# idiap/IdiapTTS

Measured on AMD Instinct MI355X. Metric: acoustic frames/sec (train), higher is better.
Workload: dtype f32

## Files before the change

idiaptts_amd/csrc/gemm_ring.h:

```cpp
#pragma once
#include <hip/hip_runtime.h>
#include <stdint.h>

#ifndef RING_DBG
#define RING_DBG 0
#endif

namespace itts {
namespace ring {

typedef float f32x16 __attribute__((ext_vector_type(16)));
typedef float f32x4 __attribute__((ext_vector_type(4)));
typedef __attribute__((address_space(3))) char* lds_char_p;

constexpr int RBK = 32;
constexpr int SLOT_BYTES = 192 * 128;
#ifndef RING_NSLOT
#define RING_NSLOT 3
#endif
constexpr int NSLOT = RING_NSLOT;
constexpr int RED_BYTES = 2 * 256 * 4;
constexpr int LDS_BYTES = NSLOT * SLOT_BYTES + RED_BYTES;
constexpr int PIECES = 6;
constexpr int THREADS = 512;

enum { EPI_STORE = 0, EPI_BIAS_ACT = 1, EPI_DACT = 2, EPI_MSE = 3 };
enum { ACT_NONE = 0, ACT_TANH = 1, ACT_RELU = 2 };

struct Args {
  const float* A;
  const float* B;
  float* C;
  const float* bias;
  const float* aux;
  const uint8_t* row_valid;
  double* loss_partial;
  float* bias_part;
  uint64_t* stamps;
  int64_t slab_stride;
  int64_t bias_part_stride;
  int lda, ldb, ldc, ldaux;
  int M;
  int N;
  int K;
  int kchunk;
  int splitk;
  int tiles_m, tiles_n;
  int gn;
  int act;
  float gscale;
};

__device__ __forceinline__ float fast_tanhf(float z) {
  const float a = fabsf(z);
  const float z2 = z * z;
  const float poly = z * (1.f + z2 * (-0.33333334f + z2 * (0.13333334f + z2 * (-0.053968254f +
                                                                              z2 * 0.021869488f))));
  const float e = __expf(2.f * a);
  const float big = copysignf(1.f - 2.f * __builtin_amdgcn_rcpf(e + 1.f), z);
  return a < 0.25f ? poly : big;
}

__device__ __forceinline__ __amdgpu_buffer_rsrc_t make_rsrc(const void* p, uint32_t bytes) {
  return __builtin_amdgcn_make_buffer_rsrc(const_cast<void*>(p), 0, (int)bytes, 0x00020000);
}

__device__ __forceinline__ void dma_piece(__amdgpu_buffer_rsrc_t rsrc, uint32_t voff, uint32_t soff, uint32_t dst) {
  asm volatile("s_nop 4\n\ts_mov_b32 m0, %3\n\ts_nop 0\n\tbuffer_load_dwordx4 %0, %1, %2 offen lds"
               :
               : "v"(voff), "s"(rsrc), "s"(soff), "s"(dst)
               : "memory");
}

__device__ __forceinline__ void lds_barrier() {
  asm volatile("s_waitcnt lgkmcnt(0)" ::: "memory");
  __builtin_amdgcn_s_barrier();
  asm volatile("" ::: "memory");
}
__device__ __forceinline__ void step_barrier() {
  if (!(RING_DBG & 2)) __builtin_amdgcn_s_barrier();
  asm volatile("" ::: "memory");
}

template <bool ROW, int BT>
__device__ __forceinline__ float4 read_frag(const char* tile, uint32_t a0, int g) {
  if (ROW) {
    return *reinterpret_cast<const float4*>(tile + (a0 ^ (uint32_t)(g << 5)));
  } else {
    const float* p = reinterpret_cast<const float*>(tile + a0) + g * 8 * BT;
    return make_float4(p[0], p[BT], p[2 * BT], p[3 * BT]);
  }
}
template <bool ROW, int BT>
__device__ __forceinline__ uint32_t frag_base(int o, int lane) {
  const int r = lane & 31, h = lane >> 5;
  if (ROW) {
    const int row = o + r;
    return (uint32_t)(row * 128 + ((((row >> 1) & 7) ^ h) << 4));
  } else {
    return (uint32_t)((4 * h * BT + o + r) * 4);
  }
}

struct Tile {
  int m0, n0, z, tn;
  int kbeg, klen, nk;
};

template <bool GROUPED>
__device__ __forceinline__ Tile decode_tile(const Args& g, int t, int bmt, int bnt) {
  Tile c;
  const int per_z = g.tiles_m * g.tiles_n;
  c.z = t / per_z;
  const int rem = t - c.z * per_z;
  int tm;
  if (!GROUPED) {
    tm = rem / g.tiles_n;
    c.tn = rem - tm * g.tiles_n;
  } else {
    const int per_group = g.tiles_m * g.gn;
    const int grp = rem / per_group;
    const int rem2 = rem - grp * per_group;
    const int left = g.tiles_n - grp * g.gn;
    const int width = left < g.gn ? left : g.gn;
    tm = rem2 / width;
    c.tn = grp * g.gn + (rem2 - tm * width);
  }
  c.m0 = tm * bmt;
  c.n0 = c.tn * bnt;
  c.kbeg = c.z * g.kchunk;
  const int kend = c.kbeg + g.kchunk < g.K ? c.kbeg + g.kchunk : g.K;
  c.klen = kend - c.kbeg;
  c.nk = (c.klen + RBK - 1) / RBK;
  return c;
}

struct Walk {
  int first, end, stride;
};
__device__ __forceinline__ Walk my_tiles(const Args& g) {
  const int ntiles = g.tiles_m * g.tiles_n * g.splitk;
  const int xcd = blockIdx.x & 7, rank = blockIdx.x >> 3;
  const int q = ntiles >> 3, r8 = ntiles & 7;
  const int xstart = xcd < r8 ? xcd * (q + 1) : r8 * (q + 1) + (xcd - r8) * q;
  Walk w;
  w.first = xstart + rank;
  w.end = xstart + q + (xcd < r8 ? 1 : 0);
  w.stride = ((int)gridDim.x - xcd + 7) >> 3;
  return w;
}

template <bool ROW, int BT>
struct Stream {
  __amdgpu_buffer_rsrc_t rsrc;
  uint32_t soff, step;

  __device__ __forceinline__ void open(const float* P, int ld, int out0, int out_dim, const Tile& c) {
    if (ROW) {
      int rows = out_dim - out0;
      rows = rows < BT ? rows : BT;
      step = RBK * 4;
      rsrc = make_rsrc(P + (int64_t)out0 * ld + c.kbeg, (uint32_t)(((int64_t)(rows - 1) * ld + ((c.klen + 3) & ~3)) * 4));
    } else {
      step = (uint32_t)(RBK * ld * 4);
      rsrc = make_rsrc(P + (int64_t)c.kbeg * ld + out0,
                       (uint32_t)(((int64_t)(c.klen - 1) * ld + ((out_dim - out0 + 3) & ~3)) * 4));
    }
    soff = 0;
  }
  __device__ __forceinline__ void issue(uint32_t v0, uint32_t v1, int ld, uint32_t dst, int part) const {
    constexpr int NP = BT / 32;
    if (ROW) {
      const uint32_t pstep = (uint32_t)(16 * ld * 4);
      uint32_t so = soff + (uint32_t)(part * (NP / 2)) * pstep;
      const uint32_t d = dst + part * NP * 1024;
#pragma unroll
      for (int j = 0; j < NP; j += 2) {
        dma_piece(rsrc, v0, so, d + j * 1024);
        dma_piece(rsrc, v1, so, d + (j + 1) * 1024);
        so += pstep;
      }
    } else {
      const uint32_t pstep = (uint32_t)((256 / BT) * ld * 4);
      uint32_t so = soff + (uint32_t)(part * NP) * pstep;
      const uint32_t d = dst + part * NP * 1024;
#pragma unroll
      for (int j = 0; j < NP; ++j) {
        dma_piece(rsrc, v0, so, d + j * 1024);
        so += pstep;
      }
    }
  }
};
template <bool ROW, int BT>
__device__ __forceinline__ void lane_offsets(int ld, int lane, uint32_t& v0, uint32_t& v1) {
  if (ROW) {
    const int r = lane >> 3, c = lane & 7;
    v0 = (uint32_t)(r * ld * 4 + ((c ^ ((r >> 1) & 7)) << 4));
    v1 = (uint32_t)((8 + r) * ld * 4 + ((c ^ (((8 + r) >> 1) & 7)) << 4));
  } else {
    constexpr int LPR = BT / 4;
    v0 = (uint32_t)((lane / LPR) * ld * 4 + (lane % LPR) * 16);
    v1 = v0;
  }
}

template <int BT>
__device__ __forceinline__ void zero_tail(char* tile, int krem, int tid) {
#pragma unroll
  for (int i = 0; i < BT / 32; ++i) {
    const int idx = tid + 256 * i;
    const int row = idx >> 3, c = idx & 7;
    const int lim = krem - 4 * c;
    if (lim < 4) {
      float4* p = reinterpret_cast<float4*>(tile + row * 128 + ((c ^ ((row >> 1) & 7)) << 4));
      float4 v = *p;
      v.x = lim > 0 ? v.x : 0.f;
      v.y = lim > 1 ? v.y : 0.f;
      v.z = lim > 2 ? v.z : 0.f;
      v.w = 0.f;
      *p = v;
    }
  }
}

template <bool A_ROW, bool B_ROW, int BMT, int BNT, bool GROUPED = false>
__device__ __forceinline__ void loader_wave(const Args& g, char* lds, uint32_t lds0, int lane, bool mse, int part) {
  constexpr int A_BYTES = BMT * 128;
  const Walk w = my_tiles(g);
  uint32_t va0, va1, vb0, vb1;
  lane_offsets<A_ROW, BMT>(g.lda, lane, va0, va1);
  lane_offsets<B_ROW, BNT>(g.ldb, lane, vb0, vb1);
  Stream<A_ROW, BMT> sa;
  Stream<B_ROW, BNT> sb;

  int pt = w.first, pk = 0, pnk = 0;
  uint32_t pdst = lds0;
  bool pvalid = pt < w.end;
  auto open = [&]() {
    const Tile c = decode_tile<GROUPED>(g, pt, BMT, BNT);
    sa.open(g.A, g.lda, c.m0, g.M, c);
    sb.open(g.B, g.ldb, c.n0, g.N, c);
    pnk = c.nk;
    pk = 0;
  };
  auto produce = [&]() {
    if (!(RING_DBG & 1)) {
      sa.issue(va0, va1, g.lda, pdst, part);
      sb.issue(vb0, vb1, g.ldb, pdst + A_BYTES, part);
    }
    pdst = pdst == lds0 + (NSLOT - 1) * SLOT_BYTES ? lds0 : pdst + SLOT_BYTES;
    sa.soff += sa.step;
    sb.soff += sb.step;
    if (++pk == pnk) {
      pt += w.stride;
      pvalid = pt < w.end;
      if (pvalid) open();
    }
  };
  int ahead = 0;
  if (pvalid) {
    open();
    for (int i = 0; i < NSLOT - 1 && pvalid; ++i) { produce(); ++ahead; }
  }
  int ct = w.first, kt = 0, cslot = 0;
  bool have = ct < w.end;
  Tile c{};
  if (have) c = decode_tile<GROUPED>(g, ct, BMT, BNT);
  while (have) {
    if (ahead >= 5) asm volatile("s_waitcnt vmcnt(%0)" ::"n"(4 * PIECES) : "memory");
    else if (ahead == 4) asm volatile("s_waitcnt vmcnt(%0)" ::"n"(3 * PIECES) : "memory");
    else if (ahead == 3) asm volatile("s_waitcnt vmcnt(%0)" ::"n"(2 * PIECES) : "memory");
    else if (ahead == 2) asm volatile("s_waitcnt vmcnt(%0)" ::"n"(PIECES) : "memory");
    else asm volatile("s_waitcnt vmcnt(0)" ::: "memory");
    step_barrier();
    --ahead;
    if (pvalid) { produce(); ++ahead; }
    if ((A_ROW || B_ROW) && kt == c.nk - 1 && (c.klen & (RBK - 1)) != 0) step_barrier();
    cslot = cslot == NSLOT - 1 ? 0 : cslot + 1;
    if (++kt == c.nk) {
      kt = 0;
      ct += w.stride;
      have = ct < w.end;
      if (have) c = decode_tile<GROUPED>(g, ct, BMT, BNT);
    }
  }
  if (w.first < w.end) step_barrier();
  if (mse) step_barrier();
}

template <int ACT>
__device__ __forceinline__ float act1(float z) {
  if (ACT == ACT_TANH) return fast_tanhf(z);
  if (ACT == ACT_RELU) return z > 0.f ? z : 0.f;
  return z;
}
template <int ACT>
__device__ __forceinline__ float dact1(float y) {
  if (ACT == ACT_TANH) return 1.f - y * y;
  if (ACT == ACT_RELU) return y > 0.f ? 1.f : 0.f;
  return 1.f;
}

template <int CTRL>
__device__ __forceinline__ float quad_swap(float v) {
  return __builtin_bit_cast(float, __builtin_amdgcn_update_dpp(0, __builtin_bit_cast(int, v), CTRL, 0xf, 0xf, true));
}
__device__ __forceinline__ float4 quad_transpose(float a0, float a1, float a2, float a3, int lane) {
  const bool odd = lane & 1, hi = lane & 2;
  const float s0 = quad_swap<0xB1>(a0), s1 = quad_swap<0xB1>(a1), s2 = quad_swap<0xB1>(a2), s3 = quad_swap<0xB1>(a3);
  const float x0 = odd ? s1 : a0, x1 = odd ? a1 : s0;
  const float x2 = odd ? s3 : a2, x3 = odd ? a3 : s2;
  const float t0 = quad_swap<0x4E>(x0), t1 = quad_swap<0x4E>(x1), t2 = quad_swap<0x4E>(x2), t3 = quad_swap<0x4E>(x3);
  return make_float4(hi ? t2 : x0, hi ? t3 : x1, hi ? x2 : t0, hi ? x3 : t1);
}

template <int EPI>
__device__ __forceinline__ float4 load_bias(const Args& g, int n0, int wn, int lane) {
  float4 bv = make_float4(0.f, 0.f, 0.f, 0.f);
  if ((EPI == EPI_BIAS_ACT || EPI == EPI_MSE) && g.bias) {
    const int col = n0 + wn * 32 + 4 * ((lane & 31) >> 2);
    const __amdgpu_buffer_rsrc_t rb = make_rsrc(g.bias, (uint32_t)(g.N * 4));
    bv.x = __builtin_bit_cast(float, __builtin_amdgcn_raw_buffer_load_b32(rb, col * 4, 0, 0));
    bv.y = __builtin_bit_cast(float, __builtin_amdgcn_raw_buffer_load_b32(rb, col * 4 + 4, 0, 0));
    bv.z = __builtin_bit_cast(float, __builtin_amdgcn_raw_buffer_load_b32(rb, col * 4 + 8, 0, 0));
    bv.w = __builtin_bit_cast(float, __builtin_amdgcn_raw_buffer_load_b32(rb, col * 4 + 12, 0, 0));
  }
  return bv;
}

template <int EPI, int ACT>
__device__ __forceinline__ void epilogue(const Args& g, const Tile& pc, const f32x16& acc0, const f32x16& acc1,
                                         int wm, int wn, int lane, const float4& bv, double& lsum) {
  const int quad = (lane & 31) >> 2, j = lane & 3, h = lane >> 5;
  const int col = pc.n0 + wn * 32 + 4 * quad;
  const int rloc = wm * 64 + 4 * h + j;
  int rows_valid = g.M - pc.m0;
  rows_valid = rows_valid < 0 ? 0 : rows_valid;
  float* Cb = g.C + (int64_t)pc.z * g.slab_stride + (int64_t)pc.m0 * g.ldc;
  const __amdgpu_buffer_rsrc_t rc = make_rsrc(Cb, (uint32_t)((int64_t)rows_valid * g.ldc * 4));
  const uint32_t cofs = col < g.ldc ? (uint32_t)((rloc * g.ldc + col) * 4) : 0xfffffff0u;
  __amdgpu_buffer_rsrc_t rx = rc;
  uint32_t xofs = 0;
  if (EPI == EPI_DACT || EPI == EPI_MSE) {
    rx = make_rsrc(g.aux + (int64_t)pc.m0 * g.ldaux, (uint32_t)((int64_t)rows_valid * g.ldaux * 4));
    xofs = col < g.ldaux ? (uint32_t)((rloc * g.ldaux + col) * 4) : 0xfffffff0u;
  }
  const bool k0 = col < g.N, k1 = col + 1 < g.N, k2 = col + 2 < g.N, k3 = col + 3 < g.N;
#pragma unroll
  for (int i = 0; i < 2; ++i) {
    const f32x16& a = i == 0 ? acc0 : acc1;
#pragma unroll
    for (int rg = 0; rg < 4; ++rg) {
      const int rl = i * 32 + 8 * rg;
      float4 v = quad_transpose(a[4 * rg], a[4 * rg + 1], a[4 * rg + 2], a[4 * rg + 3], lane);
      if (EPI == EPI_BIAS_ACT) {
        v.x = act1<ACT>(v.x + bv.x); v.y = act1<ACT>(v.y + bv.y);
        v.z = act1<ACT>(v.z + bv.z); v.w = act1<ACT>(v.w + bv.w);
      }
      if (EPI == EPI_DACT) {
        const f32x4 y = __builtin_amdgcn_raw_buffer_load_b128(rx, xofs, rl * g.ldaux * 4, 0);
        v.x *= dact1<ACT>(y[0]); v.y *= dact1<ACT>(y[1]);
        v.z *= dact1<ACT>(y[2]); v.w *= dact1<ACT>(y[3]);
      }
      if (EPI == EPI_MSE) {
        f32x4 t;
        {
          const uint32_t so = (uint32_t)(rl * g.ldaux * 4);
          const uint32_t tofs = (uint32_t)((rloc * g.ldaux + col) * 4);
          t[0] = __builtin_bit_cast(float, __builtin_amdgcn_raw_buffer_load_b32(rx, tofs, so, 0));
          t[1] = __builtin_bit_cast(float, __builtin_amdgcn_raw_buffer_load_b32(rx, tofs + 4, so, 0));
          t[2] = __builtin_bit_cast(float, __builtin_amdgcn_raw_buffer_load_b32(rx, tofs + 8, so, 0));
          t[3] = __builtin_bit_cast(float, __builtin_amdgcn_raw_buffer_load_b32(rx, tofs + 12, so, 0));
        }
        const int row = pc.m0 + rloc + rl;
        const bool ok = row < g.M && g.row_valid[row < g.M ? row : 0] != 0;
        const float d0 = ok && k0 ? (v.x + bv.x) - t[0] : 0.f;
        const float d1 = ok && k1 ? (v.y + bv.y) - t[1] : 0.f;
        const float d2 = ok && k2 ? (v.z + bv.z) - t[2] : 0.f;
        const float d3 = ok && k3 ? (v.w + bv.w) - t[3] : 0.f;
        lsum += (double)d0 * (double)d0;
        lsum += (double)d1 * (double)d1;
        lsum += (double)d2 * (double)d2;
        lsum += (double)d3 * (double)d3;
        v = make_float4(g.gscale * d0, g.gscale * d1, g.gscale * d2, g.gscale * d3);
      }
      f32x4 o;
      o[0] = k0 ? v.x : 0.f;
      o[1] = k1 ? v.y : 0.f;
      o[2] = k2 ? v.z : 0.f;
      o[3] = k3 ? v.w : 0.f;
      const uint32_t vo = col < g.ldc ? cofs + (uint32_t)(rl * g.ldc * 4) : 0xfffffff0u;
      if (RING_DBG & 64) asm volatile("" ::"v"(o[0]), "v"(o[1]), "v"(o[2]), "v"(o[3]));
      else __builtin_amdgcn_raw_buffer_store_b128(o, rc, vo, 0, 0);
    }
  }
}

template <bool A_ROW, bool B_ROW, int EPI, int BMT, int BNT, bool GROUPED = false>
__device__ __forceinline__ void compute_waves(const Args& g, char* lds, int wid, int lane) {
  constexpr int WN = BNT / 32;
  constexpr int A_BYTES = BMT * 128;
  const int wm = wid / WN, wn = wid % WN;
  const int tid = wid * 64 + lane;
  const Walk w = my_tiles(g);
  const uint32_t fa0 = frag_base<A_ROW, BMT>(wm * 64, lane);
  const uint32_t fa1 = frag_base<A_ROW, BMT>(wm * 64 + 32, lane);
  const uint32_t fb0 = frag_base<B_ROW, BNT>(wn * 32, lane);
  float* red = reinterpret_cast<float*>(lds + NSLOT * SLOT_BYTES);
  constexpr bool DO_BIAS = !A_ROW && EPI == EPI_STORE;
  constexpr int BPARTS = 256 / BMT;

  double lsum = 0.0;
  int cslot = 0, redbuf = 0;
  bool pending = false;
  Tile pc{};
  f32x16 acc0, acc1;
#pragma unroll
  for (int r = 0; r < 16; ++r) { acc0[r] = 0.f; acc1[r] = 0.f; }
  float bsum = 0.f;

  int ct = w.first;
  bool have = ct < w.end;
  Tile c{};
  if (have) c = decode_tile<GROUPED>(g, ct, BMT, BNT);
  int kt = 0;
  while (have || pending) {
    step_barrier();
    if (pending) {
      if (DO_BIAS && g.bias_part != nullptr && pc.tn == 0) {
        const float* rb = red + (redbuf ^ 1) * 256;
        if (tid < BMT && pc.m0 + tid < g.M) {
          float s = rb[tid];
#pragma unroll
          for (int p = 1; p < BPARTS; ++p) s += rb[tid + p * BMT];
          g.bias_part[(int64_t)pc.z * g.bias_part_stride + pc.m0 + tid] = s;
        }
      }
      if (RING_DBG & 8) {
        float t = 0.f;
        for (int r = 0; r < 16; ++r) t += acc0[r] + acc1[r];
        if (t == 1.2345f) g.C[0] = t;
      } else {
        const float4 bv = load_bias<EPI>(g, pc.n0, wn, lane);
        if (EPI == EPI_STORE || g.act == ACT_NONE) epilogue<EPI, ACT_NONE>(g, pc, acc0, acc1, wm, wn, lane, bv, lsum);
        else if (g.act == ACT_TANH) epilogue<EPI, ACT_TANH>(g, pc, acc0, acc1, wm, wn, lane, bv, lsum);
        else epilogue<EPI, ACT_RELU>(g, pc, acc0, acc1, wm, wn, lane, bv, lsum);
      }
      pending = false;
    }
    if (!have) break;

    char* tA = lds + cslot * SLOT_BYTES;
    char* tB = tA + A_BYTES;
    if ((A_ROW || B_ROW) && kt == c.nk - 1 && (c.klen & (RBK - 1)) != 0) {
      if (A_ROW) zero_tail<BMT>(tA, c.klen & (RBK - 1), tid);
      if (B_ROW) zero_tail<BNT>(tB, c.klen & (RBK - 1), tid);
      lds_barrier();
    }
    if (DO_BIAS && g.bias_part != nullptr && c.tn == 0) {
      constexpr int KP = RBK / BPARTS;
      const float* ctile = reinterpret_cast<const float*>(tA) + (tid / BMT) * KP * BMT + tid % BMT;
#pragma unroll
      for (int kk = 0; kk < KP; ++kk) bsum += ctile[kk * BMT];
    }
#pragma unroll
    for (int kg = 0; kg < 4; ++kg) {
      float4 a0, a1, b0;
      if (RING_DBG & 16) {
        a0 = make_float4(1.f + kg, 2.f, 3.f, 4.f); a1 = a0; b0 = a0;
        asm volatile("" : "+v"(a0.x), "+v"(a1.x), "+v"(b0.x));
      } else {
        a0 = read_frag<A_ROW, BMT>(tA, fa0, kg);
        a1 = read_frag<A_ROW, BMT>(tA, fa1, kg);
        b0 = read_frag<B_ROW, BNT>(tB, fb0, kg);
      }
      if (RING_DBG & 4) {
        asm volatile("" ::"v"(a0.x), "v"(a0.y), "v"(a0.z), "v"(a0.w), "v"(a1.x), "v"(a1.y), "v"(a1.z), "v"(a1.w),
                     "v"(b0.x), "v"(b0.y), "v"(b0.z), "v"(b0.w));
        continue;
      }
      if (kg == 0 && kt == 0) {
        const f32x16 zero = {0.f, 0.f, 0.f, 0.f, 0.f, 0.f, 0.f, 0.f, 0.f, 0.f, 0.f, 0.f, 0.f, 0.f, 0.f, 0.f};
        acc0 = __builtin_amdgcn_mfma_f32_32x32x2f32(a0.x, b0.x, zero, 0, 0, 0);
        acc1 = __builtin_amdgcn_mfma_f32_32x32x2f32(a1.x, b0.x, zero, 0, 0, 0);
      } else {
        acc0 = __builtin_amdgcn_mfma_f32_32x32x2f32(a0.x, b0.x, acc0, 0, 0, 0);
        acc1 = __builtin_amdgcn_mfma_f32_32x32x2f32(a1.x, b0.x, acc1, 0, 0, 0);
      }
      acc0 = __builtin_amdgcn_mfma_f32_32x32x2f32(a0.y, b0.y, acc0, 0, 0, 0);
      acc1 = __builtin_amdgcn_mfma_f32_32x32x2f32(a1.y, b0.y, acc1, 0, 0, 0);
      acc0 = __builtin_amdgcn_mfma_f32_32x32x2f32(a0.z, b0.z, acc0, 0, 0, 0);
      acc1 = __builtin_amdgcn_mfma_f32_32x32x2f32(a1.z, b0.z, acc1, 0, 0, 0);
      acc0 = __builtin_amdgcn_mfma_f32_32x32x2f32(a0.w, b0.w, acc0, 0, 0, 0);
      acc1 = __builtin_amdgcn_mfma_f32_32x32x2f32(a1.w, b0.w, acc1, 0, 0, 0);
    }
    cslot = cslot == NSLOT - 1 ? 0 : cslot + 1;
    if (++kt == c.nk) {
      if (DO_BIAS && g.bias_part != nullptr && c.tn == 0) {
        red[redbuf * 256 + tid] = bsum;
        bsum = 0.f;
        redbuf ^= 1;
        asm volatile("s_waitcnt lgkmcnt(0)" ::: "memory");
      }
      pending = true;
      pc = c;
      kt = 0;
      ct += w.stride;
      have = ct < w.end;
      if (have) c = decode_tile<GROUPED>(g, ct, BMT, BNT);
    }
  }
  if (EPI == EPI_MSE) {
    double* redd = reinterpret_cast<double*>(red);
#pragma unroll
    for (int off = 32; off > 0; off >>= 1) lsum += __shfl_xor(lsum, off, 64);
    if (lane == 0) redd[wid] = lsum;
    lds_barrier();
    if (tid == 0) g.loss_partial[blockIdx.x] = (redd[0] + redd[1]) + (redd[2] + redd[3]);
  }
}

template <bool A_ROW, bool B_ROW, int EPI, int WM, bool GROUPED = false>
__global__ __launch_bounds__(THREADS, (2 * THREADS + 255) / 256) void gemm_ring_kernel(Args g) {
  constexpr int BMT = 64 * WM, BNT = 32 * (4 / WM);
  __shared__ __attribute__((aligned(1024))) char lds[LDS_BYTES];
  const uint32_t lds0 = (uint32_t)(uintptr_t)(lds_char_p)lds;
  const int lane = threadIdx.x & 63;
  const int wid = __builtin_amdgcn_readfirstlane(threadIdx.x >> 6);
  uint64_t t0c = 0, t0r = 0;
  if (g.stamps) { t0c = __builtin_amdgcn_s_memtime(); t0r = __builtin_amdgcn_s_memrealtime(); }
  if (wid >= 4) {
    loader_wave<A_ROW, B_ROW, BMT, BNT, GROUPED>(g, lds, lds0, lane, EPI == EPI_MSE, wid - 4);
  } else {
    compute_waves<A_ROW, B_ROW, EPI, BMT, BNT, GROUPED>(g, lds, wid, lane);
  }
  if (g.stamps && threadIdx.x == 0) {
    g.stamps[4 * blockIdx.x] = __builtin_amdgcn_s_memtime() - t0c;
    g.stamps[4 * blockIdx.x + 1] = __builtin_amdgcn_s_memrealtime() - t0r;
    g.stamps[4 * blockIdx.x + 2] = t0r;
  }
}

template <bool A1, bool B1, int E1, int W1, bool A2, bool B2, int E2, int W2>
__global__ __launch_bounds__(THREADS, (2 * THREADS + 255) / 256) void gemm_ring_pair_kernel(Args g1, Args g2) {
  __shared__ __attribute__((aligned(1024))) char lds[LDS_BYTES];
  const uint32_t lds0 = (uint32_t)(uintptr_t)(lds_char_p)lds;
  const int lane = threadIdx.x & 63;
  const int wid = __builtin_amdgcn_readfirstlane(threadIdx.x >> 6);
  if (wid >= 4) {
    loader_wave<A1, B1, 64 * W1, 32 * (4 / W1)>(g1, lds, lds0, lane, E1 == EPI_MSE, wid - 4);
    loader_wave<A2, B2, 64 * W2, 32 * (4 / W2)>(g2, lds, lds0, lane, E2 == EPI_MSE, wid - 4);
  } else {
    compute_waves<A1, B1, E1, 64 * W1, 32 * (4 / W1)>(g1, lds, wid, lane);
    compute_waves<A2, B2, E2, 64 * W2, 32 * (4 / W2)>(g2, lds, wid, lane);
  }
}

}
}
```

Measured before the change: 37.65 million.

## Prefetch epilogue aux/target loads during main K loop to hide latency

For the DACT and MSE epilogues, the aux activation and target tiles are now loaded into registers a couple of K-steps before the tile finishes, instead of being loaded inside the epilogue after the MMA loop. The row-valid mask is fetched once per lane and broadcast with a shuffle rather than read per row from global memory. This is meant to overlap epilogue global-load latency with MFMA compute. The cost is extra registers held across the loop (8 float4 per lane), which may lower occupancy or cause spills. A debug flag to skip the tail barrier and zeroing is also added.

```diff
diff --git a/idiaptts_amd/csrc/gemm_ring.h b/idiaptts_amd/csrc/gemm_ring.h
--- a/idiaptts_amd/csrc/gemm_ring.h
+++ b/idiaptts_amd/csrc/gemm_ring.h
@@ -276,7 +276,7 @@
     step_barrier();
     --ahead;
     if (pvalid) { produce(); ++ahead; }
-    if ((A_ROW || B_ROW) && kt == c.nk - 1 && (c.klen & (RBK - 1)) != 0) step_barrier();
+    if (!(RING_DBG & 128) && (A_ROW || B_ROW) && kt == c.nk - 1 && (c.klen & (RBK - 1)) != 0) step_barrier();
     cslot = cslot == NSLOT - 1 ? 0 : cslot + 1;
     if (++kt == c.nk) {
       kt = 0;
@@ -315,37 +315,63 @@
   return make_float4(hi ? t2 : x0, hi ? t3 : x1, hi ? x2 : t0, hi ? x3 : t1);
 }
 
+constexpr int EPI_LEAD = 2;
+__device__ __forceinline__ int epi_fetch_step(int nk) { return nk > EPI_LEAD + 1 ? nk - EPI_LEAD : (nk > 1 ? 1 : 0); }
 template <int EPI>
-__device__ __forceinline__ float4 load_bias(const Args& g, int n0, int wn, int lane) {
-  float4 bv = make_float4(0.f, 0.f, 0.f, 0.f);
+struct EpiIn {
+  float4 bias;
+  f32x4 x[(EPI == EPI_DACT || EPI == EPI_MSE) ? 8 : 1];
+  int ok;
+};
+
+__device__ __forceinline__ int epi_col(const Tile& c, int wn, int lane) { return c.n0 + wn * 32 + 4 * ((lane & 31) >> 2); }
+__device__ __forceinline__ int epi_rloc(int wm, int lane) { return wm * 64 + 4 * (lane >> 5) + (lane & 3); }
+__device__ __forceinline__ int epi_rows(const Args& g, const Tile& c) { return g.M - c.m0 < 0 ? 0 : g.M - c.m0; }
+
+template <int EPI>
+__device__ __forceinline__ void epi_fetch(const Args& g, const Tile& c, int wm, int wn, int lane, EpiIn<EPI>& in) {
+  const int col = epi_col(c, wn, lane), rloc = epi_rloc(wm, lane);
+  in.bias = make_float4(0.f, 0.f, 0.f, 0.f);
   if ((EPI == EPI_BIAS_ACT || EPI == EPI_MSE) && g.bias) {
-    const int col = n0 + wn * 32 + 4 * ((lane & 31) >> 2);
     const __amdgpu_buffer_rsrc_t rb = make_rsrc(g.bias, (uint32_t)(g.N * 4));
-    bv.x = __builtin_bit_cast(float, __builtin_amdgcn_raw_buffer_load_b32(rb, col * 4, 0, 0));
-    bv.y = __builtin_bit_cast(float, __builtin_amdgcn_raw_buffer_load_b32(rb, col * 4 + 4, 0, 0));
-    bv.z = __builtin_bit_cast(float, __builtin_amdgcn_raw_buffer_load_b32(rb, col * 4 + 8, 0, 0));
-    bv.w = __builtin_bit_cast(float, __builtin_amdgcn_raw_buffer_load_b32(rb, col * 4 + 12, 0, 0));
-  }
-  return bv;
+    in.bias.x = __builtin_bit_cast(float, __builtin_amdgcn_raw_buffer_load_b32(rb, col * 4, 0, 0));
+    in.bias.y = __builtin_bit_cast(float, __builtin_amdgcn_raw_buffer_load_b32(rb, col * 4 + 4, 0, 0));
+    in.bias.z = __builtin_bit_cast(float, __builtin_amdgcn_raw_buffer_load_b32(rb, col * 4 + 8, 0, 0));
+    in.bias.w = __builtin_bit_cast(float, __builtin_amdgcn_raw_buffer_load_b32(rb, col * 4 + 12, 0, 0));
+  }
+  if (EPI == EPI_DACT || EPI == EPI_MSE) {
+    const __amdgpu_buffer_rsrc_t rx =
+        make_rsrc(g.aux + (int64_t)c.m0 * g.ldaux, (uint32_t)((int64_t)epi_rows(g, c) * g.ldaux * 4));
+#pragma unroll
+    for (int q = 0; q < 8; ++q) {
+      const int rl = (q >> 2) * 32 + 8 * (q & 3);
+      const uint32_t so = (uint32_t)(rl * g.ldaux * 4);
+      if (EPI == EPI_DACT) {
+        const uint32_t xofs = col < g.ldaux ? (uint32_t)((rloc * g.ldaux + col) * 4) : 0xfffffff0u;
+        in.x[q] = __builtin_amdgcn_raw_buffer_load_b128(rx, xofs, so, 0);
+      } else {
+        const uint32_t tofs = (uint32_t)((rloc * g.ldaux + col) * 4);
+        in.x[q][0] = __builtin_bit_cast(float, __builtin_amdgcn_raw_buffer_load_b32(rx, tofs, so, 0));
+        in.x[q][1] = __builtin_bit_cast(float, __builtin_amdgcn_raw_buffer_load_b32(rx, tofs + 4, so, 0));
+        in.x[q][2] = __builtin_bit_cast(float, __builtin_amdgcn_raw_buffer_load_b32(rx, tofs + 8, so, 0));
+        in.x[q][3] = __builtin_bit_cast(float, __builtin_amdgcn_raw_buffer_load_b32(rx, tofs + 12, so, 0));
+      }
+    }
+  }
+  if (EPI == EPI_MSE) {
+    const __amdgpu_buffer_rsrc_t rv = make_rsrc(g.row_valid + c.m0, (uint32_t)epi_rows(g, c));
+    in.ok = __builtin_amdgcn_raw_buffer_load_b8(rv, wm * 64 + lane, 0, 0);
+  }
 }
 
 template <int EPI, int ACT>
 __device__ __forceinline__ void epilogue(const Args& g, const Tile& pc, const f32x16& acc0, const f32x16& acc1,
-                                         int wm, int wn, int lane, const float4& bv, double& lsum) {
-  const int quad = (lane & 31) >> 2, j = lane & 3, h = lane >> 5;
-  const int col = pc.n0 + wn * 32 + 4 * quad;
-  const int rloc = wm * 64 + 4 * h + j;
-  int rows_valid = g.M - pc.m0;
-  rows_valid = rows_valid < 0 ? 0 : rows_valid;
+                                         int wm, int wn, int lane, const EpiIn<EPI>& in, double& lsum) {
+  const int col = epi_col(pc, wn, lane), rloc = epi_rloc(wm, lane);
+  const float4 bv = in.bias;
   float* Cb = g.C + (int64_t)pc.z * g.slab_stride + (int64_t)pc.m0 * g.ldc;
-  const __amdgpu_buffer_rsrc_t rc = make_rsrc(Cb, (uint32_t)((int64_t)rows_valid * g.ldc * 4));
+  const __amdgpu_buffer_rsrc_t rc = make_rsrc(Cb, (uint32_t)((int64_t)epi_rows(g, pc) * g.ldc * 4));
   const uint32_t cofs = col < g.ldc ? (uint32_t)((rloc * g.ldc + col) * 4) : 0xfffffff0u;
-  __amdgpu_buffer_rsrc_t rx = rc;
-  uint32_t xofs = 0;
-  if (EPI == EPI_DACT || EPI == EPI_MSE) {
-    rx = make_rsrc(g.aux + (int64_t)pc.m0 * g.ldaux, (uint32_t)((int64_t)rows_valid * g.ldaux * 4));
-    xofs = col < g.ldaux ? (uint32_t)((rloc * g.ldaux + col) * 4) : 0xfffffff0u;
-  }
   const bool k0 = col < g.N, k1 = col + 1 < g.N, k2 = col + 2 < g.N, k3 = col + 3 < g.N;
 #pragma unroll
   for (int i = 0; i < 2; ++i) {
@@ -359,22 +385,13 @@
         v.z = act1<ACT>(v.z + bv.z); v.w = act1<ACT>(v.w + bv.w);
       }
       if (EPI == EPI_DACT) {
-        const f32x4 y = __builtin_amdgcn_raw_buffer_load_b128(rx, xofs, rl * g.ldaux * 4, 0);
+        const f32x4 y = in.x[4 * i + rg];
         v.x *= dact1<ACT>(y[0]); v.y *= dact1<ACT>(y[1]);
         v.z *= dact1<ACT>(y[2]); v.w *= dact1<ACT>(y[3]);
       }
       if (EPI == EPI_MSE) {
-        f32x4 t;
-        {
-          const uint32_t so = (uint32_t)(rl * g.ldaux * 4);
-          const uint32_t tofs = (uint32_t)((rloc * g.ldaux + col) * 4);
-          t[0] = __builtin_bit_cast(float, __builtin_amdgcn_raw_buffer_load_b32(rx, tofs, so, 0));
-          t[1] = __builtin_bit_cast(float, __builtin_amdgcn_raw_buffer_load_b32(rx, tofs + 4, so, 0));
-          t[2] = __builtin_bit_cast(float, __builtin_amdgcn_raw_buffer_load_b32(rx, tofs + 8, so, 0));
-          t[3] = __builtin_bit_cast(float, __builtin_amdgcn_raw_buffer_load_b32(rx, tofs + 12, so, 0));
-        }
-        const int row = pc.m0 + rloc + rl;
-        const bool ok = row < g.M && g.row_valid[row < g.M ? row : 0] != 0;
+        const f32x4 t = in.x[4 * i + rg];
+        const bool ok = __shfl(in.ok, rloc - wm * 64 + rl, 64) != 0;
         const float d0 = ok && k0 ? (v.x + bv.x) - t[0] : 0.f;
         const float d1 = ok && k1 ? (v.y + bv.y) - t[1] : 0.f;
         const float d2 = ok && k2 ? (v.z + bv.z) - t[2] : 0.f;
@@ -415,6 +432,7 @@
   int cslot = 0, redbuf = 0;
   bool pending = false;
   Tile pc{};
+  EpiIn<EPI> ein;
   f32x16 acc0, acc1;
 #pragma unroll
   for (int r = 0; r < 16; ++r) { acc0[r] = 0.f; acc1[r] = 0.f; }
@@ -442,10 +460,10 @@
         for (int r = 0; r < 16; ++r) t += acc0[r] + acc1[r];
         if (t == 1.2345f) g.C[0] = t;
       } else {
-        const float4 bv = load_bias<EPI>(g, pc.n0, wn, lane);
-        if (EPI == EPI_STORE || g.act == ACT_NONE) epilogue<EPI, ACT_NONE>(g, pc, acc0, acc1, wm, wn, lane, bv, lsum);
-        else if (g.act == ACT_TANH) epilogue<EPI, ACT_TANH>(g, pc, acc0, acc1, wm, wn, lane, bv, lsum);
-        else epilogue<EPI, ACT_RELU>(g, pc, acc0, acc1, wm, wn, lane, bv, lsum);
+        if (EPI == EPI_BIAS_ACT) epi_fetch<EPI>(g, pc, wm, wn, lane, ein);
+        if (EPI == EPI_STORE || g.act == ACT_NONE) epilogue<EPI, ACT_NONE>(g, pc, acc0, acc1, wm, wn, lane, ein, lsum);
+        else if (g.act == ACT_TANH) epilogue<EPI, ACT_TANH>(g, pc, acc0, acc1, wm, wn, lane, ein, lsum);
+        else epilogue<EPI, ACT_RELU>(g, pc, acc0, acc1, wm, wn, lane, ein, lsum);
       }
       pending = false;
     }
@@ -453,11 +471,13 @@
 
     char* tA = lds + cslot * SLOT_BYTES;
     char* tB = tA + A_BYTES;
-    if ((A_ROW || B_ROW) && kt == c.nk - 1 && (c.klen & (RBK - 1)) != 0) {
+    if (!(RING_DBG & 128) && (A_ROW || B_ROW) && kt == c.nk - 1 && (c.klen & (RBK - 1)) != 0) {
       if (A_ROW) zero_tail<BMT>(tA, c.klen & (RBK - 1), tid);
       if (B_ROW) zero_tail<BNT>(tB, c.klen & (RBK - 1), tid);
       lds_barrier();
     }
+    if ((EPI == EPI_DACT || EPI == EPI_MSE) && !(RING_DBG & 8) && kt == epi_fetch_step(c.nk))
+      epi_fetch<EPI>(g, c, wm, wn, lane, ein);
     if (DO_BIAS && g.bias_part != nullptr && c.tn == 0) {
       constexpr int KP = RBK / BPARTS;
       const float* ctile = reinterpret_cast<const float*>(tA) + (tid / BMT) * KP * BMT + tid % BMT;
```

Result: faster. 38.20 million (median of 6 runs) (+1.5%).
